# ZhangYY12345/aswStereoMatch

Measured on AMD Instinct MI355X. Metric: disparity Mpix/s, 1920x1080 D=128 classic bilateral ASW (computeAdaptiveWeight), higher is better.
Workload: dtype f64; 1 GPU; 1920x1080 D=128 win=15 bilateral, 8 frames/GPU/step resident in HBM, cost volume kept; candidates=129, parallelism=frames sharded, no collective, ranks=1, backend=none

## Files before the change

aswstereomatch_amd/csrc/k_bilateral_xq.hip:

```cpp
#include <stdlib.h>

#include <algorithm>
#include <cmath>

#include "asw_device.h"
#include "asw_internal.h"

namespace {

constexpr int HH = 7;
constexpr int KS = 2 * HH + 1;
constexpr int PXW = 64;
constexpr int LWC = PXW + 2 * HH;
constexpr int NSTEP = KS + 3;
constexpr int RING = 5;
constexpr int URI = 3;
constexpr int CROW = 6;
static_assert(KS % URI == 0 && CROW % URI == 0, "whole bodies");
constexpr int NCELLCOL = NSTEP + 3;
constexpr int LW8 = 80;
constexpr int LWP = 80;

template <int NW>
struct XqCfg {
    static constexpr int NWAVE = NW;
    static constexpr int NTHR = 64 * NW;
    static constexpr int NJ = 4 * NW;
    static constexpr int NPOS = PXW + 4 * NJ;
    static constexpr int RWC = NPOS + 2 * HH;
    static constexpr int NFIN = 4 * NJ;
    static constexpr int RW8 = (RWC + 3) / 4 * 4;
    static constexpr int NROWS = (KS + NW - 1) / NW;
    static constexpr int RWP = (RWC + 3) / 4 * 4;
    static constexpr int LROW = RING * PXW + LWP;
    static constexpr int RROW = 2 * NPOS + RWP;
    static constexpr int LGRAY = RING * PXW;
    static constexpr int RGRAY = 2 * NPOS;
    static constexpr int OFF_LB = 0;
    static constexpr int OFF_RB = OFF_LB + KS * LROW * 4;
    static constexpr int OFF_L8 = OFF_RB + KS * RROW * 4;
    static constexpr int OFF_R8 = OFF_L8 + KS * LW8;
    static constexpr int OFF_CELL = OFF_R8 + KS * RW8;
    static constexpr int OFF_E64 = 0;
    static constexpr int OFF_PART = NFIN * PXW * 8;
    static constexpr int LDS_TOTAL = std::max((OFF_CELL + NCELLCOL * KS * 2 + 15) / 16 * 16, OFF_PART + NW * PXW * 12);
    static_assert(LDS_TOTAL <= (NW == 8 ? 80 : 53) * 1024, "two (NW = 8) / three (NW = 4) workgroups per CU");
    static_assert(OFF_RB % 16 == 0 && (LROW * 4) % 16 == 0 && (RROW * 4) % 16 == 0 && (NPOS * 4) % 16 == 0 && (LGRAY * 4) % 16 == 0, "b128 alignment");
    static_assert(NPOS % 64 == 0, "positions are staged in whole wavefront passes");
};
#define XQ_CONSTS(NW)                                                                                                           \
    typedef XqCfg<NW> Cfg;                                                                                                       \
    constexpr int NWAVE = Cfg::NWAVE, NTHR = Cfg::NTHR, NJ = Cfg::NJ, NPOS = Cfg::NPOS, RWC = Cfg::RWC, NFIN = Cfg::NFIN, RW8 = Cfg::RW8,      \
                  NROWS = Cfg::NROWS, LROW = Cfg::LROW, RROW = Cfg::RROW, LGRAY = Cfg::LGRAY, RGRAY = Cfg::RGRAY,               \
                  OFF_LB = Cfg::OFF_LB, OFF_RB = Cfg::OFF_RB, OFF_L8 = Cfg::OFF_L8, OFF_R8 = Cfg::OFF_R8, OFF_CELL = Cfg::OFF_CELL,  \
                  LDS_TOTAL = Cfg::LDS_TOTAL, OFF_E64 = Cfg::OFF_E64, OFF_PART = Cfg::OFF_PART;                                  \
    (void)NWAVE; (void)NTHR; (void)NJ; (void)NPOS; (void)RWC; (void)NFIN; (void)RW8; (void)NROWS; (void)LROW; (void)RROW; (void)LGRAY;  \
    (void)RGRAY; (void)OFF_LB; (void)OFF_RB; (void)OFF_L8; (void)OFF_R8; (void)OFF_CELL; (void)LDS_TOTAL; (void)OFF_E64; (void)OFF_PART;

struct XqParams {
    int H, W, minD;
    int tile0;
};

__device__ __forceinline__ double cost_sample(uint32_t gl, uint32_t gr, uint32_t hi0)
{
    const uint32_t c = __builtin_amdgcn_sad_u16(gl, gr, 0u);
    return __builtin_bit_cast(double, (uint64_t)c | ((uint64_t)hi0 << 32));
}

template <int NW>
__device__ __forceinline__ void cell_at(const unsigned char* smem, int idx, int& dxw, int& dyw, int& cls256)
{
    XQ_CONSTS(NW)
    const uint32_t u = reinterpret_cast<const uint16_t*>(smem + OFF_CELL)[idx];
    dxw = (int)(u & 15u) - 8;
    dyw = (int)((u >> 4) & 15u) - 8;
    cls256 = (int)(u >> 8) << 8;
}

template <int NW> struct Staged { float v[XqCfg<NW>::NROWS][1 + XqCfg<NW>::NPOS / 64]; };

template <int NW>
__device__ __forceinline__ void stage_issue(int Kn, const float* __restrict__ lut, const unsigned char* smem, int wave, int lane,
                                            uint32_t ppack, Staged<NW>& st)
{
    XQ_CONSTS(NW)
    const uint8_t* sL8 = smem + OFF_L8;
    const uint8_t* sR8 = smem + OFF_R8;
#pragma unroll
    for (int rr = 0; rr < NROWS; rr++) {
        const int ky = wave + NWAVE * rr;
        if (ky >= KS) break;
        int dxw, dyw, cls;
        if (Kn < KS) {
            cell_at<NW>(smem, (Kn + 3) * KS + ky, dxw, dyw, cls);
            const int nb = sL8[(HH + dyw) * LW8 + (lane + HH + dxw)];
            st.v[rr][0] = lut_at(lut, __builtin_amdgcn_sad_u16(nb, sL8[HH * LW8 + lane + HH], cls));
        }
#pragma unroll
        for (int r3 = 0; r3 < NPOS / 64; r3++) {
            const int b = lane & 3;
            cell_at<NW>(smem, (Kn - b + 3) * KS + ky, dxw, dyw, cls);
            const int pc = (int)((ppack >> (8 * r3)) & 255u) + HH;
            const int ctr = sR8[HH * RW8 + pc];
            const int nb = sR8[(HH + dyw) * RW8 + pc + dxw];
            st.v[rr][1 + r3] = lut_at(lut, __builtin_amdgcn_sad_u16(nb, ctr, cls));
        }
    }
}

template <int NW>
__device__ __forceinline__ void stage_commit(int Kn, unsigned char* smem, int wave, int lane, const Staged<NW>& st)
{
    XQ_CONSTS(NW)
    float* sWL = reinterpret_cast<float*>(smem + OFF_LB) + (Kn % RING) * PXW;
    float* sWR = reinterpret_cast<float*>(smem + OFF_RB) + (Kn & 1) * NPOS;
#pragma unroll
    for (int rr = 0; rr < NROWS; rr++) {
        const int ky = wave + NWAVE * rr;
        if (ky >= KS) break;
        if (Kn < KS) sWL[ky * LROW + lane] = st.v[rr][0];
#pragma unroll
        for (int r3 = 0; r3 < NPOS / 64; r3++) sWR[ky * RROW + lane + 64 * r3] = st.v[rr][1 + r3];
    }
}

template <int NW>
__device__ __forceinline__ void stage_weights(int Kn, const float* __restrict__ lut, unsigned char* smem, int wave, int lane,
                                              uint32_t ppack)
{
    Staged<NW> st;
    stage_issue<NW>(Kn, lut, smem, wave, lane, ppack, st);
    stage_commit<NW>(Kn, smem, wave, lane, st);
}

template <int NW, int K, bool EDGE, bool WRAPW, bool COMMIT, bool RIGHT>
__device__ __forceinline__ void run_step(unsigned char* smem, int g, int qrel, int qrel2, int xabs, int dbase, int dbase2,
                                         int W, int x0, int posmin, double (&num)[4][4], double (&den)[4][4], int wave, int lane,
                                         const Staged<NW>& st)
{
    XQ_CONSTS(NW)
    constexpr int BLO = K > KS - 1 ? K - (KS - 1) : 0;
    constexpr int BHI = K < 3 ? K : 3;
    constexpr int DLO = 0 - BHI, DHI = 3 - BLO;
    const uint32_t* sLd = reinterpret_cast<const uint32_t*>(smem + OFF_LB) + LGRAY;
    const uint32_t* sRd = reinterpret_cast<const uint32_t*>(smem + OFF_RB) + RGRAY;

    int iL[7], iR[7];
    if constexpr (EDGE) {
#pragma unroll
        for (int dl = DLO; dl <= DHI; dl++) {
            const int lc = min(max(xabs + dl + K - HH, 0), W - 1);
            const int rc = RIGHT ? lc + ((dl > 0 ? dbase2 : dbase) - dl) : lc - ((dl < 0 ? dbase2 : dbase) + dl);
            iL[dl + 3] = min(max(lc - (x0 - HH), 0), LWC - 1);
            iR[dl + 3] = min(max(rc - (posmin - HH), 0), RWC - 1);
        }
    }
    typedef __attribute__((address_space(3))) const unsigned char lds_u8;
    lds_u8* bL = (lds_u8*)smem + OFF_LB + 16 * g;
    lds_u8* bR = (lds_u8*)smem + OFF_RB + 4 * qrel;
    lds_u8* bR2 = (lds_u8*)smem + OFF_RB + 4 * qrel2;
    uint32_t hi0[7];
#pragma unroll
    for (int i = 0; i < 7; i++) asm volatile("v_mov_b32 %0, 0" : "=v"(hi0[i]));
    constexpr int UR = EDGE ? 1 : URI;
    auto rows = [&](int ky0, int nbody) {
#pragma unroll 1
        for (int it = 0; it < nbody; it++) {
#pragma unroll
            for (int u = 0; u < UR; u++) {
                lds_u8* rL = bL + u * 4 * LROW;
                lds_u8* rR = bR + u * 4 * RROW;
                lds_u8* rR2 = bR2 + u * 4 * RROW;
                double c[7];
                if constexpr (!EDGE) {
                    const uint32_t gr = *(const __attribute__((address_space(3))) uint32_t*)(rR + 4 * (RGRAY + K));
                    uint32_t gr2 = gr;
                    if constexpr (WRAPW && (RIGHT ? DHI > 0 : DLO < 0)) gr2 = *(const __attribute__((address_space(3))) uint32_t*)(rR2 + 4 * (RGRAY + K));
                    constexpr int E0 = (K + DLO) & ~3, NQ = (K + DHI - E0 + 4) / 4;
                    static_assert(E0 >= 0 && E0 + 4 * NQ + 4 * 15 <= LWP, "the quads stay inside a tile row");
                    typedef uint32_t u32x4 __attribute__((ext_vector_type(4)));
                    const __attribute__((address_space(3))) u32x4* pl4 = (const __attribute__((address_space(3))) u32x4*)(rL + 4 * (LGRAY + E0));
                    uint32_t glv[4 * NQ];
#pragma unroll
                    for (int i = 0; i < NQ; i++) {
                        u32x4 t = pl4[i];
                        asm("" : "+v"(t));
                        glv[4 * i] = t.x; glv[4 * i + 1] = t.y; glv[4 * i + 2] = t.z; glv[4 * i + 3] = t.w;
                    }
#pragma unroll
                    for (int dl = DLO; dl <= DHI; dl++) c[dl + 3] = cost_sample(glv[K + dl - E0], (RIGHT ? dl > 0 : dl < 0) ? gr2 : gr, hi0[dl + 3]);
                } else {
                    const int ky = ky0 + it * UR + u;
#pragma unroll
                    for (int dl = DLO; dl <= DHI; dl++) c[dl + 3] = cost_sample(sLd[ky * LROW + iL[dl + 3]], sRd[ky * RROW + iR[dl + 3]], hi0[dl + 3]);
                }
                typedef float f32x4 __attribute__((ext_vector_type(4)));
                typedef __attribute__((address_space(3))) const f32x4 lds_f32x4;
                const f32x4 wr4 = *(lds_f32x4*)(rR + 4 * (K & 1) * NPOS);
                typedef float f32x2 __attribute__((ext_vector_type(2)));
                f32x2 wrp[2] = {{wr4.x, wr4.y}, {wr4.z, wr4.w}};
                asm("" : "+v"(wrp[1]));
                f32x2 wr2p[2] = {wrp[0], wrp[1]};
                if constexpr ((WRAPW || EDGE) && (RIGHT ? BLO <= 2 : BHI >= 1)) {
                    const f32x4 w2 = *(lds_f32x4*)(rR2 + 4 * (K & 1) * NPOS);
                    wr2p[0] = f32x2{w2.x, w2.y};
                    wr2p[1] = f32x2{w2.z, w2.w};
                    asm("" : "+v"(wr2p[1]));
                }
#pragma unroll
                for (int b = BLO; b <= BHI; b++) {
                    const f32x4 wl4 = *(lds_f32x4*)(rL + 4 * ((K - b) % RING) * PXW);
                    float ab[4];
#pragma unroll
                    for (int a = 0; a < 4; a += 2) {
                        const f32x2 wl2 = {wl4[a], wl4[a + 1]};
                        const bool w0 = RIGHT ? b < a : a < b, w1 = RIGHT ? b < a + 1 : a + 1 < b;
                        const f32x2 s0 = (w0 ? wr2p : wrp)[b >> 1], s1 = (w1 ? wr2p : wrp)[b >> 1];
                        f32x2 wrb;
                        if (w0 == w1) wrb = (b & 1) ? __builtin_shufflevector(s0, s0, 1, 1) : __builtin_shufflevector(s0, s0, 0, 0);
                        else wrb = f32x2{s0[b & 1], s1[b & 1]};
                        const f32x2 pr = wl2 * wrb;
                        ab[a] = pr.x; ab[a + 1] = pr.y;
                    }
#pragma unroll
                    for (int a = 0; a < 4; a++) {
                        const double abd = (double)ab[a];
                        num[a][b] = __builtin_fma(abd, c[a - b + 3], num[a][b]);
                        den[a][b] = den[a][b] + abd;
                    }
                }
#pragma unroll
                for (int b = BLO; b <= BHI; b++)
                    asm volatile("" :: "v"(num[0][b]), "v"(num[1][b]), "v"(num[2][b]), "v"(num[3][b]),
                                       "v"(den[0][b]), "v"(den[1][b]), "v"(den[2][b]), "v"(den[3][b]) : "memory");
                __builtin_amdgcn_sched_barrier(0);
            }
            bL += UR * 4 * LROW;
            bR += UR * 4 * RROW;
            asm("" : "+v"(bL), "+v"(bR));
            if constexpr (WRAPW || EDGE) {
                bR2 += UR * 4 * RROW;
                asm("" : "+v"(bR2));
            }
        }
    };
    if constexpr (COMMIT) {
        rows(0, CROW / UR);
        stage_commit<NW>(K + 1, smem, wave, lane, st);
        rows(CROW, (KS - CROW) / UR);
    } else {
        rows(0, KS / UR);
    }
}

template <int NW, bool EDGE, bool WRAPW, int ABL, bool RIGHT>
__device__ __forceinline__ void run_all_steps(unsigned char* smem, const float* __restrict__ lut, int wave, int lane,
                                              uint32_t ppack, int g, int qrel, int qrel2, int xabs, int dbase, int dbase2,
                                              int W, int x0, int posmin, double (&num)[4][4], double (&den)[4][4])
{
    Staged<NW> st;
#define ASW_XQ_STEP(KK)                                                                                        \
    if (!(ABL & 1) && (KK) + 1 < NSTEP) {                                                                        \
        if constexpr (EDGE) stage_weights<NW>((KK) + 1, lut, smem, wave, lane, ppack);   \
        else stage_issue<NW>((KK) + 1, lut, smem, wave, lane, ppack, st);                      \
    }                                                                                                           \
    run_step<NW, (KK), EDGE, WRAPW, (!EDGE && !(ABL & 1) && (KK) + 1 < NSTEP), RIGHT>(smem, g, qrel, qrel2, xabs, dbase, dbase2, W, x0, posmin, \
                                                                           num, den, wave, lane, st);          \
    if (!(ABL & 2) || (KK) == NSTEP - 1) __syncthreads();
    ASW_XQ_STEP(0) ASW_XQ_STEP(1) ASW_XQ_STEP(2) ASW_XQ_STEP(3) ASW_XQ_STEP(4) ASW_XQ_STEP(5)
    ASW_XQ_STEP(6) ASW_XQ_STEP(7) ASW_XQ_STEP(8) ASW_XQ_STEP(9) ASW_XQ_STEP(10) ASW_XQ_STEP(11)
    ASW_XQ_STEP(12) ASW_XQ_STEP(13) ASW_XQ_STEP(14) ASW_XQ_STEP(15) ASW_XQ_STEP(16) ASW_XQ_STEP(17)
#undef ASW_XQ_STEP
}

template <int NW, bool EDGE, int ABL, bool RIGHT>
__global__ __launch_bounds__(64 * NW) __attribute__((amdgpu_waves_per_eu(NW == 8 ? 4 : 3, NW == 8 ? 4 : 3))) void k_asw_bilateral_xq(
    XqParams p, const uint8_t* __restrict__ gL, const uint8_t* __restrict__ gR, const int4* __restrict__ cells,
    const float* __restrict__ lut, float* __restrict__ vol, double* __restrict__ bestE, float* __restrict__ bestD,
    float* __restrict__ disp)
{
    XQ_CONSTS(NW)
    __shared__ __align__(16) unsigned char smem[LDS_TOTAL];
    const int tid = threadIdx.x, lane = tid & 63, wave = __builtin_amdgcn_readfirstlane(tid >> 6);
    const int H = p.H, W = p.W;
    const int x0 = (p.tile0 + blockIdx.x) * PXW, y = blockIdx.y;
    const int posmin = RIGHT ? x0 + p.minD : x0 - p.minD - 4 * NJ;

    {
        uint8_t* sL8 = smem + OFF_L8;
        uint8_t* sR8 = smem + OFF_R8;
        uint32_t* sLd = reinterpret_cast<uint32_t*>(smem + OFF_LB) + Cfg::LGRAY;
        uint32_t* sRd = reinterpret_cast<uint32_t*>(smem + OFF_RB) + Cfg::RGRAY;
        for (int i = tid; i < KS * LWC; i += NTHR) {
            const int r = i / LWC, c = i - r * LWC;
            const int yy = min(max(y - HH + r, 0), H - 1), xx = min(max(x0 - HH + c, 0), W - 1);
            const int v = gL[(size_t)yy * W + xx];
            sL8[r * LW8 + c] = (uint8_t)v;
            sLd[r * Cfg::LROW + c] = (uint32_t)v;
        }
        for (int i = tid; i < KS * RWC; i += NTHR) {
            const int r = i / RWC, c = i - r * RWC;
            const int yy = min(max(y - HH + r, 0), H - 1), xx = min(max(posmin - HH + c, 0), W - 1);
            const int v = gR[(size_t)yy * W + xx];
            sR8[r * RW8 + c] = (uint8_t)v;
            sRd[r * Cfg::RROW + c] = (uint32_t)v;
        }
        uint16_t* sCell = reinterpret_cast<uint16_t*>(smem + OFF_CELL);
        for (int i = tid; i < NCELLCOL * KS; i += NTHR) {
            const int4 ci = cells[i];
            sCell[i] = (uint16_t)((uint32_t)(ci.x + 8) | ((uint32_t)(ci.y + 8) << 4) | ((uint32_t)(ci.z >> 8) << 8));
        }
    }
    __syncthreads();

    const int g = (lane & 7) | ((lane >> 2) & 8);
    const int jl = 4 * wave + ((lane >> 3) & 3);
    const int qrel = RIGHT ? 4 * g + 4 * jl : 4 * g + 4 * (NJ - jl);
    const int qrel2 = jl == 0 ? (RIGHT ? 4 * g + 4 * NJ : 4 * g) : qrel;
    const int xabs = x0 + 4 * g;
    const int dbase = p.minD + 4 * jl;
    const int dbase2 = jl == 0 ? p.minD + 4 * NJ : dbase;
    const int pclamp_lo = min(max(0 - posmin, 0), NPOS - 1), pclamp_hi = min(max(W - 1 - posmin, 0), NPOS - 1);
    static_assert(NPOS <= 256, "a clamped position fits a byte");
    uint32_t ppack = 0;
#pragma unroll
    for (int r3 = 0; r3 < NPOS / 64; r3++) ppack |= (uint32_t)min(max(lane + 64 * r3, pclamp_lo), pclamp_hi) << (8 * r3);
    asm volatile("" : "+v"(ppack));

    double num[4][4], den[4][4];
#pragma unroll
    for (int a = 0; a < 4; a++)
#pragma unroll
        for (int b = 0; b < 4; b++) { num[a][b] = 0.0; den[a][b] = 0.0; }

    stage_weights<NW>(0, lut, smem, wave, lane, ppack);
    __syncthreads();
    if (EDGE || wave == 0)
        run_all_steps<NW, EDGE, true, ABL, RIGHT>(smem, lut, wave, lane, ppack, g, qrel, qrel2, xabs, dbase, dbase2, W,
                                                   x0, posmin, num, den);
    else
        run_all_steps<NW, EDGE, false, ABL, RIGHT>(smem, lut, wave, lane, ppack, g, qrel, qrel2, xabs, dbase, dbase2, W,
                                                    x0, posmin, num, den);

    int le = lane;
    asm volatile("" : "+v"(le));
    const int ge = (le & 7) | ((le >> 2) & 8), jle = 4 * wave + ((le >> 3) & 3);
    const int cb = 4 * jle, cb2 = jle == 0 ? 4 * NJ : cb;
    double* sE = reinterpret_cast<double*>(smem + OFF_E64);
#pragma unroll
    for (int a = 0; a < 4; a++)
#pragma unroll
        for (int b = 0; b < 4; b++) {
            const int c = RIGHT ? (b < a ? cb2 : cb) + b - a : (a < b ? cb2 : cb) + a - b;
            sE[c * PXW + 4 * ge + a] = __builtin_ldexp(num[a][b], 954) / __builtin_ldexp(den[a][b], -120);
        }
    __syncthreads();
    const int px = lane, part = wave;
    const int x = x0 + px;
    double be = 1.7976931348623157e308;
    float bd = 0.0f;
    if (x < W) {
        for (int c = 16 * part; c < 16 * part + 16; c++) {
            const double E = sE[c * PXW + px];
            if (vol) vol[((size_t)c * H + y) * W + x] = (float)E;
            if (E < be) { be = E; bd = (float)(p.minD + c); }
        }
    }
    double* sPE = reinterpret_cast<double*>(smem + OFF_PART);
    float* sPD = reinterpret_cast<float*>(smem + OFF_PART + NWAVE * PXW * 8);
    sPE[part * PXW + px] = be;
    sPD[part * PXW + px] = bd;
    __syncthreads();
    if (wave == 0 && x < W) {
        double e = 1.7976931348623157e308;
        float d = 0.0f;
#pragma unroll
        for (int q = 0; q < NWAVE; q++) {
            const double eq = sPE[q * PXW + px];
            if (eq < e) { e = eq; d = sPD[q * PXW + px]; }
        }
        if (disp) {
            disp[(size_t)y * W + x] = d;
        } else {
            bestE[(size_t)y * W + x] = e;
            bestD[(size_t)y * W + x] = d;
        }
    }
}

}

int bilateral_xq_candidates(int nwave) { return 16 * nwave; }

bool bilateral_xq_lut_ok(const float* lut, size_t n)
{
    double mn = 0, mx = 0;
    for (size_t i = 0; i < n; i++) {
        const double v = lut[i];
        if (!(v >= 0)) return false;
        if (v > 0 && (mn == 0 || v < mn)) mn = v;
        if (v > mx) mx = v;
    }
    return mn * mn >= std::ldexp(1.0, -68) && mx * mx < std::ldexp(1.0, 128 - 2 * XQ_LUT_SCALE_LOG2 - 1);
}

namespace {
template <int NW>
int launch_xq_t(hipStream_t s, hipStream_t s_border, const uint8_t* gL, const uint8_t* gR, int H, int W, int minD, const int4* cells,
                const float* lut, float* vol, double* bestE, float* bestD, float* disp, bool right)
{
    const int ntiles = (W + PXW - 1) / PXW;
    const dim3 blk(64 * NW);
    if (right) {
        if ((ntiles - 1) * PXW + minD > W - 1) return ASW_ERR_BAD_ARGUMENT;
        XqParams pe{H, W, minD, 0};
        hipLaunchKernelGGL((k_asw_bilateral_xq<NW, true, 0, true>), dim3(1, H), blk, 0, s_border, pe, gL, gR, cells, lut, vol,
                           bestE, bestD, disp);
        if (ntiles > 1) {
            XqParams pi{H, W, minD, 1};
            hipLaunchKernelGGL((k_asw_bilateral_xq<NW, false, 0, true>), dim3(ntiles - 1, H), blk, 0, s, pi, gL, gR, cells, lut,
                               vol, bestE, bestD, disp);
        }
        ASW_HIP_TRY(hipGetLastError());
        return ASW_OK;
    }
    const int n_int = W >= PXW + HH ? std::min(ntiles, (W - PXW - HH) / PXW + 1) : 0;
#ifdef ASW_XQ_ABLATION
    int abl = 0;
    if (const char* e = getenv("ASW_XQ_ABLATE")) abl = atoi(e) & 3;
    auto ki = abl == 0 ? k_asw_bilateral_xq<NW, false, 0, false> : abl == 1 ? k_asw_bilateral_xq<NW, false, 1, false>
            : abl == 2 ? k_asw_bilateral_xq<NW, false, 2, false> : k_asw_bilateral_xq<NW, false, 3, false>;
#else
    auto ki = k_asw_bilateral_xq<NW, false, 0, false>;
#endif
    auto ke = k_asw_bilateral_xq<NW, true, 0, false>;
    if (n_int > 0) {
        XqParams p{H, W, minD, 0};
        hipLaunchKernelGGL(ki, dim3(n_int, H), blk, 0, s, p, gL, gR, cells, lut, vol, bestE, bestD, disp);
    }
    if (ntiles > n_int) {
        XqParams p{H, W, minD, n_int};
        hipLaunchKernelGGL(ke, dim3(ntiles - n_int, H), blk, 0, s_border, p, gL, gR, cells, lut, vol, bestE, bestD, disp);
    }
    ASW_HIP_TRY(hipGetLastError());
    return ASW_OK;
}
}

int launch_bilateral_xq(hipStream_t s, hipStream_t s_border, int nwave, const uint8_t* gL, const uint8_t* gR, int H, int W, int minD,
                        const int4* cells, const float* lut, float* vol, double* bestE, float* bestD, float* disp, bool right)
{
    if (nwave == 8) return launch_xq_t<8>(s, s_border, gL, gR, H, W, minD, cells, lut, vol, bestE, bestD, disp, right);
    if (nwave == 4) return launch_xq_t<4>(s, s_border, gL, gR, H, W, minD, cells, lut, vol, bestE, bestD, disp, right);
    return ASW_ERR_BAD_ARGUMENT;
}
```

Baseline: 244.3 Mpix/s.

## Batch tile-load global reads in registers and precompute cell LDS offsets

The prologue now has each wave load its image rows into registers, all global loads issued up front, before any LDS store. The old loop interleaved loads and stores with integer divides. The cell table is split into three u16 arrays: precomputed left offsets, right offsets and class bases. This drops the per-sample unpack and multiply-add in the staging loop at the cost of three times the cell LDS footprint and more registers held during the prologue.

```diff
diff --git a/aswstereomatch_amd/csrc/k_bilateral_xq.hip b/aswstereomatch_amd/csrc/k_bilateral_xq.hip
--- a/aswstereomatch_amd/csrc/k_bilateral_xq.hip
+++ b/aswstereomatch_amd/csrc/k_bilateral_xq.hip
@@ -18,6 +18,7 @@
 constexpr int CROW = 6;
 static_assert(KS % URI == 0 && CROW % URI == 0, "whole bodies");
 constexpr int NCELLCOL = NSTEP + 3;
+constexpr int NCELL = NCELLCOL * KS;
 constexpr int LW8 = 80;
 constexpr int LWP = 80;
 
@@ -43,10 +44,11 @@
     static constexpr int OFF_CELL = OFF_R8 + KS * RW8;
     static constexpr int OFF_E64 = 0;
     static constexpr int OFF_PART = NFIN * PXW * 8;
-    static constexpr int LDS_TOTAL = std::max((OFF_CELL + NCELLCOL * KS * 2 + 15) / 16 * 16, OFF_PART + NW * PXW * 12);
+    static constexpr int LDS_TOTAL = std::max((OFF_CELL + 3 * NCELL * 2 + 15) / 16 * 16, OFF_PART + NW * PXW * 12);
     static_assert(LDS_TOTAL <= (NW == 8 ? 80 : 53) * 1024, "two (NW = 8) / three (NW = 4) workgroups per CU");
     static_assert(OFF_RB % 16 == 0 && (LROW * 4) % 16 == 0 && (RROW * 4) % 16 == 0 && (NPOS * 4) % 16 == 0 && (LGRAY * 4) % 16 == 0, "b128 alignment");
     static_assert(NPOS % 64 == 0, "positions are staged in whole wavefront passes");
+    static_assert(OFF_CELL % 2 == 0 && KS * RW8 <= 65536 && KS * LW8 <= 65536, "the cell table's offsets are u16");
 };
 #define XQ_CONSTS(NW)                                                                                                           \
     typedef XqCfg<NW> Cfg;                                                                                                       \
@@ -69,13 +71,19 @@
 }
 
 template <int NW>
-__device__ __forceinline__ void cell_at(const unsigned char* smem, int idx, int& dxw, int& dyw, int& cls256)
+__device__ __forceinline__ uint16_t cell_entry(int4 ci, int side)
+{
+    const int stride = side == 0 ? LW8 : XqCfg<NW>::RW8;
+    return (uint16_t)(side == 2 ? (ci.z >> 8) << 8 : (HH + ci.y) * stride + HH + ci.x);
+}
+
+template <int NW, bool RSIDE>
+__device__ __forceinline__ void cell_at(const unsigned char* smem, int idx, int& off, int& cls256)
 {
     XQ_CONSTS(NW)
-    const uint32_t u = reinterpret_cast<const uint16_t*>(smem + OFF_CELL)[idx];
-    dxw = (int)(u & 15u) - 8;
-    dyw = (int)((u >> 4) & 15u) - 8;
-    cls256 = (int)(u >> 8) << 8;
+    const uint16_t* t = reinterpret_cast<const uint16_t*>(smem + OFF_CELL);
+    off = t[(RSIDE ? NCELL : 0) + idx];
+    cls256 = t[2 * NCELL + idx];
 }
 
 template <int NW> struct Staged { float v[XqCfg<NW>::NROWS][1 + XqCfg<NW>::NPOS / 64]; };
@@ -91,19 +99,19 @@
     for (int rr = 0; rr < NROWS; rr++) {
         const int ky = wave + NWAVE * rr;
         if (ky >= KS) break;
-        int dxw, dyw, cls;
+        int off, cls;
         if (Kn < KS) {
-            cell_at<NW>(smem, (Kn + 3) * KS + ky, dxw, dyw, cls);
-            const int nb = sL8[(HH + dyw) * LW8 + (lane + HH + dxw)];
+            cell_at<NW, false>(smem, (Kn + 3) * KS + ky, off, cls);
+            const int nb = sL8[off + lane];
             st.v[rr][0] = lut_at(lut, __builtin_amdgcn_sad_u16(nb, sL8[HH * LW8 + lane + HH], cls));
         }
 #pragma unroll
         for (int r3 = 0; r3 < NPOS / 64; r3++) {
             const int b = lane & 3;
-            cell_at<NW>(smem, (Kn - b + 3) * KS + ky, dxw, dyw, cls);
-            const int pc = (int)((ppack >> (8 * r3)) & 255u) + HH;
-            const int ctr = sR8[HH * RW8 + pc];
-            const int nb = sR8[(HH + dyw) * RW8 + pc + dxw];
+            cell_at<NW, true>(smem, (Kn - b + 3) * KS + ky, off, cls);
+            const int pc = (int)((ppack >> (8 * r3)) & 255u);
+            const int ctr = sR8[HH * RW8 + HH + pc];
+            const int nb = sR8[off + pc];
             st.v[rr][1 + r3] = lut_at(lut, __builtin_amdgcn_sad_u16(nb, ctr, cls));
         }
     }
@@ -288,28 +296,62 @@
     const int posmin = RIGHT ? x0 + p.minD : x0 - p.minD - 4 * NJ;
 
     {
+        constexpr int NLJ = (LWC + 63) / 64, NRJ = (RWC + 63) / 64, NCJ = (NCELL + NTHR - 1) / NTHR;
+        uint32_t xl[NLJ], xr[NRJ];
+#pragma unroll
+        for (int j = 0; j < NLJ; j++) xl[j] = (uint32_t)min(max(x0 - HH + lane + 64 * j, 0), W - 1);
+#pragma unroll
+        for (int j = 0; j < NRJ; j++) xr[j] = (uint32_t)min(max(posmin - HH + lane + 64 * j, 0), W - 1);
+        uint32_t vl[NROWS][NLJ], vr[NROWS][NRJ];
+        int4 ci[NCJ];
+#pragma unroll
+        for (int k = 0; k < NROWS; k++) {
+            const int yy = min(max(y - HH + wave + NWAVE * k, 0), H - 1);
+            const uint8_t* rowL = gL + (size_t)yy * W;
+            const uint8_t* rowR = gR + (size_t)yy * W;
+#pragma unroll
+            for (int j = 0; j < NLJ; j++) vl[k][j] = rowL[xl[j]];
+#pragma unroll
+            for (int j = 0; j < NRJ; j++) vr[k][j] = rowR[xr[j]];
+        }
+#pragma unroll
+        for (int j = 0; j < NCJ; j++) ci[j] = cells[min(tid + NTHR * j, NCELL - 1)];
         uint8_t* sL8 = smem + OFF_L8;
         uint8_t* sR8 = smem + OFF_R8;
         uint32_t* sLd = reinterpret_cast<uint32_t*>(smem + OFF_LB) + Cfg::LGRAY;
         uint32_t* sRd = reinterpret_cast<uint32_t*>(smem + OFF_RB) + Cfg::RGRAY;
-        for (int i = tid; i < KS * LWC; i += NTHR) {
-            const int r = i / LWC, c = i - r * LWC;
-            const int yy = min(max(y - HH + r, 0), H - 1), xx = min(max(x0 - HH + c, 0), W - 1);
-            const int v = gL[(size_t)yy * W + xx];
-            sL8[r * LW8 + c] = (uint8_t)v;
-            sLd[r * Cfg::LROW + c] = (uint32_t)v;
-        }
-        for (int i = tid; i < KS * RWC; i += NTHR) {
-            const int r = i / RWC, c = i - r * RWC;
-            const int yy = min(max(y - HH + r, 0), H - 1), xx = min(max(posmin - HH + c, 0), W - 1);
-            const int v = gR[(size_t)yy * W + xx];
-            sR8[r * RW8 + c] = (uint8_t)v;
-            sRd[r * Cfg::RROW + c] = (uint32_t)v;
+#pragma unroll
+        for (int part = 1; part >= 0; part--) {
+#pragma unroll
+            for (int k = 0; k < NROWS; k++) {
+                const int r = wave + NWAVE * k;
+                if (r >= KS) break;
+#pragma unroll
+                for (int j = 0; j < NLJ; j++) {
+                    const int c = lane + 64 * j;
+                    if ((64 * j + 64 > LWC) == (part == 1) && c < LWC) {
+                        sL8[r * LW8 + c] = (uint8_t)vl[k][j];
+                        sLd[r * Cfg::LROW + c] = vl[k][j];
+                    }
+                }
+#pragma unroll
+                for (int j = 0; j < NRJ; j++) {
+                    const int c = lane + 64 * j;
+                    if ((64 * j + 64 > RWC) == (part == 1) && c < RWC) {
+                        sR8[r * RW8 + c] = (uint8_t)vr[k][j];
+                        sRd[r * Cfg::RROW + c] = vr[k][j];
+                    }
+                }
+            }
         }
         uint16_t* sCell = reinterpret_cast<uint16_t*>(smem + OFF_CELL);
-        for (int i = tid; i < NCELLCOL * KS; i += NTHR) {
-            const int4 ci = cells[i];
-            sCell[i] = (uint16_t)((uint32_t)(ci.x + 8) | ((uint32_t)(ci.y + 8) << 4) | ((uint32_t)(ci.z >> 8) << 8));
+#pragma unroll
+        for (int j = 0; j < NCJ; j++) {
+            const int i = tid + NTHR * j;
+            if (i < NCELL) {
+#pragma unroll
+                for (int side = 0; side < 3; side++) sCell[side * NCELL + i] = cell_entry<NW>(ci[j], side);
+            }
         }
     }
     __syncthreads();
```

Measured after the change: 245.9 Mpix/s (median of 6 runs). About the same (+0.7%).
